# robinhenry/gym-anm

Hardware: AMD Instinct MI355X
Metric: env-steps/sec (whole node) at num_envs=65536, ANM6Easy; NR iters to 1e-6 (higher is better)
Workload: dtype f64

## Files before the change

### gym_anm_amd/csrc/anm_device.hpp

```cpp
#pragma once

#include <cmath>
#include <cstdint>
#include <type_traits>

#if defined(__HIPCC__)
#define ANM_HD __host__ __device__ __forceinline__
#define ANM_CONST_AS __attribute__((address_space(4)))
#else
#define ANM_HD inline
#define ANM_CONST_AS
#endif

#if defined(ANM_PHASE_TIMING) && defined(__HIPCC__)
#define ANM_N_PHASES 8
#define ANM_MAX_WAVES 16384
__device__ unsigned long long g_anm_phase[ANM_N_PHASES][ANM_MAX_WAVES];
#endif
#if defined(ANM_PHASE_TIMING) && defined(__HIP_DEVICE_COMPILE__)
#define ANM_PHASE(k)                                                                         \
  do {                                                                                       \
    if ((threadIdx.x & 63) == 0 && blockIdx.x < ANM_MAX_WAVES)                               \
      g_anm_phase[k][blockIdx.x] = __builtin_readcyclecounter();                             \
  } while (0)
#else
#define ANM_PHASE(k) do { } while (0)
#endif

#if defined(__HIPCC__)
#define ANM_WAVE_SYNC()                                        \
  do {                                                         \
    __builtin_amdgcn_fence(__ATOMIC_RELEASE, "wavefront");     \
    __builtin_amdgcn_wave_barrier();                           \
    __builtin_amdgcn_fence(__ATOMIC_ACQUIRE, "wavefront");     \
  } while (0)
#endif

namespace anm {

typedef const ANM_CONST_AS double* cptr_t;

template <int B, int E, class F>
ANM_HD void static_for(F&& f) {
  if constexpr (B < E) {
    f(std::integral_constant<int, B>{});
    static_for<B + 1, E>(f);
  }
}

#if defined(__HIP_DEVICE_COMPILE__)
#define ANM_WAVE_ANY(x) __any(x)
#else
#define ANM_WAVE_ANY(x) (x)
#endif

enum DevType : int { DEV_LOAD = -1, DEV_SLACK = 0, DEV_CLASSICAL = 1, DEV_RENEWABLE = 2, DEV_STORAGE = 3 };

constexpr double SINCOS_MEDIUM_MAX = 3.5e15;
ANM_HD int lo_word(double x) {
#if defined(__HIP_DEVICE_COMPILE__)
  return __double2loint(x);
#else
  unsigned long long u;
  __builtin_memcpy(&u, &x, 8);
  return int(unsigned(u));
#endif
}
ANM_HD double flip_sign(double x, unsigned m) {
#if defined(__HIP_DEVICE_COMPILE__)
  return __hiloint2double(__double2hiint(x) ^ int(m & 0x80000000u), __double2loint(x));
#else
  unsigned long long u;
  __builtin_memcpy(&u, &x, 8);
  u ^= (unsigned long long)(m & 0x80000000u) << 32;
  __builtin_memcpy(&x, &u, 8);
  return x;
#endif
}

template <bool NEG>
ANM_HD double fma3(double a, double b, double c) {
#if defined(__HIP_DEVICE_COMPILE__)
  double r;
  if constexpr (NEG) asm("v_fma_f64 %0, %1, %2, -%3" : "=v"(r) : "v"(a), "v"(b), "v"(c));
  else asm("v_fma_f64 %0, %1, %2, %3" : "=v"(r) : "v"(a), "v"(b), "v"(c));
  return r;
#else
  return fma(a, b, NEG ? -c : c);
#endif
}

template <bool VCOEF = false>
ANM_HD void sincos_kernel(double r, int q, double& s_out, double& c_out) {
  const double z = r * r;
  double sn, cs;
#if defined(__HIP_DEVICE_COMPILE__)
  if constexpr (VCOEF) {
    double ps, pc;
    asm("v_fma_f64 %0, %2, %3, %4\n\t"
        "v_fma_f64 %1, %2, %9, %10\n\t"
        "v_fma_f64 %0, %2, %0, %5\n\t"
        "v_fma_f64 %1, %2, %1, %11\n\t"
        "v_fma_f64 %0, %2, %0, %6\n\t"
        "v_fma_f64 %1, %2, %1, %12\n\t"
        "v_fma_f64 %0, %2, %0, %7\n\t"
        "v_fma_f64 %1, %2, %1, %13\n\t"
        "v_fma_f64 %0, %2, %0, %8\n\t"
        "v_fma_f64 %1, %2, %1, %14"
        : "=&v"(ps), "=&v"(pc)
        : "v"(z), "v"(1.58969099521155010221e-10), "v"(-2.50507602534068634195e-08), "v"(2.75573137070700676789e-06),
          "v"(-1.98412698298579493134e-04), "v"(8.33333333332248946124e-03), "v"(-1.66666666666666324348e-01),
          "v"(-1.13596475577881948265e-11), "v"(2.08757232129817482790e-09), "v"(-2.75573143513906633035e-07),
          "v"(2.48015872894767294178e-05), "v"(-1.38888888888741095749e-03), "v"(4.16666666666666019037e-02));
    sn = fma(r * z, ps, r);
    cs = fma(z * z, pc, fma(-0.5, z, 1.0));
  } else
#endif
  {
    double ps = fma(z, 1.58969099521155010221e-10, -2.50507602534068634195e-08);
    ps = fma(z, ps, 2.75573137070700676789e-06);
    ps = fma(z, ps, -1.98412698298579493134e-04);
    ps = fma(z, ps, 8.33333333332248946124e-03);
    ps = fma(z, ps, -1.66666666666666324348e-01);
    sn = fma(r * z, ps, r);
    double pc = fma(z, -1.13596475577881948265e-11, 2.08757232129817482790e-09);
    pc = fma(z, pc, -2.75573143513906633035e-07);
    pc = fma(z, pc, 2.48015872894767294178e-05);
    pc = fma(z, pc, -1.38888888888741095749e-03);
    pc = fma(z, pc, 4.16666666666666019037e-02);
    cs = fma(z * z, pc, fma(-0.5, z, 1.0));
  }
  const bool swap = (q & 1) != 0;
  const double a = swap ? cs : sn, b = swap ? sn : cs;
  s_out = flip_sign(a, unsigned(q) << 30);
  c_out = flip_sign(b, unsigned(q + 1) << 30);
}


ANM_HD void reduce_medium(double x, double& r_out, int& q_out) {
  const double TWO_OVER_PI = 6.36619772367581382433e-01;
  const double P1 = 1.57079632679489655800e+00, P2 = 6.12323399573676603587e-17, P3 = 1.49738490485916983e-33;
  const double fn = rint(x * TWO_OVER_PI);
  double r = fma(-fn, P1, x);
  r = fma(-fn, P2, r);
  r = fma(-fn, P3, r);
  const double f2 = rint(r * TWO_OVER_PI);
  r = fma(-f2, P1, r);
  r = fma(-f2, P2, r);
  r_out = r;
  q_out = lo_word((fn + f2) + 6755399441055744.0);
}
struct SinCos {
  double s, c;
};
#if defined(__HIPCC__)
__host__ __device__ __attribute__((noinline))
#else
inline
#endif
SinCos sincos_huge(double x) {
  SinCos r;
  sincos(x, &r.s, &r.c);
  return r;
}

template <bool VCOEF = false>
ANM_HD void sincos_medium(double x, double& s_out, double& c_out) {
  double r;
  int q;
  reduce_medium(x, r, q);
  sincos_kernel<VCOEF>(r, q, s_out, c_out);
}

enum SetDevField : int {
  SD_PMIN = 0, SD_PMAX, SD_QMIN, SD_QMAX,
  SD_SOC_MIN, SD_SOC_MAX, SD_EFF, SD_PAD,
  SD_HLO_LO, SD_HLO_HI,
  SD_HHI_LO, SD_HHI_HI,
  SD_SL,
  SD_SIZE = SD_SL + 4 * 6
};
enum SlField : int { SL_TAU = 0, SL_RHO, SL_INV, SL_LO, SL_HI, SL_SENSE };

template <class T>
struct Layout {
  static constexpr int SCALARS = 0;
  static constexpr int N_SCALARS = 8;
  static constexpr int Y_RE = SCALARS + N_SCALARS;
  static constexpr int Y_IM = Y_RE + T::NNZ;
  static constexpr int BUS_VMIN = Y_IM + T::NNZ;
  static constexpr int BUS_VMAX = BUS_VMIN + T::NB;
  static constexpr int BR = BUS_VMAX + T::NB;
  static constexpr int BR_STRIDE = 9;
  static constexpr int LOAD = BR + T::NBR * BR_STRIDE;
  static constexpr int SETDEV = LOAD + T::NLOAD * 3;
  static constexpr int KMAX = 8;
  static constexpr int OBS_LO = SETDEV + T::NSET * SD_SIZE;
  static constexpr int OBS_HI = OBS_LO + T::SDIM + KMAX;
  static constexpr int TOTAL = OBS_HI + T::SDIM + KMAX;
};
enum ScalarField : int { SC_BASE = 0, SC_DT, SC_LAMB, SC_C1, SC_C2, SC_RTERM, SC_PERIOD, SC_SPARE };

#if defined(__HIP_DEVICE_COMPILE__)
ANM_HD double vmax(double a, double b) { double r; asm("v_max_f64 %0, %1, %2" : "=v"(r) : "v"(a), "v"(b)); return r; }
ANM_HD double vmin(double a, double b) { double r; asm("v_min_f64 %0, %1, %2" : "=v"(r) : "v"(a), "v"(b)); return r; }
#else
ANM_HD double vmax(double a, double b) { return fmax(a, b); }
ANM_HD double vmin(double a, double b) { return fmin(a, b); }
#endif

template <int NSL, class SD>
ANM_HD void project_pq(SD sd, double p0, double q0, double pl, double pu, double& p_out, double& q_out) {
  const double ql = sd[SD_QMIN], qu = sd[SD_QMAX];
  const double EPS = 1e-12;
  double best_d = INFINITY, bp = p0, bq = q0;
  bool any_viol = false;

  auto consider = [&](bool violated, bool valid, double cp, double cq) {
    any_viol = any_viol || violated;
    const double dp = cp - p0, dq = cq - q0;
    const double d = dp * dp + dq * dq;
    const bool take = violated && valid && (d < best_d);
    best_d = take ? d : best_d;
    bp = take ? cp : bp;
    bq = take ? cq : bq;
  };

  auto vertical = [&](bool violated, double c) {
    double lo = ql, hi = qu;
    static_for<0, NSL>([&](auto K) {
      constexpr int k = K;
      const double tau = sd[SD_SL + 6 * k + SL_TAU], rho = sd[SD_SL + 6 * k + SL_RHO];
      const double sense = sd[SD_SL + 6 * k + SL_SENSE];
      const double v = tau * c + rho;
      hi = (sense > 0.0) ? vmin(hi, v) : hi;
      lo = (sense < 0.0) ? vmax(lo, v) : lo;
    });
    const bool valid = lo <= hi + EPS;
    const double t = vmin(vmax(q0, lo), hi);
    consider(violated, valid, c, t);
  };
  vertical(p0 < pl, pl);
  vertical(p0 > pu, pu);

  auto horizontal = [&](bool violated, double c, double slo, double shi) {
    const double lo = vmax(pl, slo), hi = vmin(pu, shi);
    const bool valid = lo <= hi + EPS;
    const double t = vmin(vmax(p0, lo), hi);
    consider(violated, valid, t, c);
  };
  horizontal(q0 < ql, ql, sd[SD_HLO_LO], sd[SD_HLO_HI]);
  horizontal(q0 > qu, qu, sd[SD_HHI_LO], sd[SD_HHI_HI]);

  static_for<0, NSL>([&](auto K) {
    constexpr int k = K;
    const double tau = sd[SD_SL + 6 * k + SL_TAU], rho = sd[SD_SL + 6 * k + SL_RHO];
    const double inv = sd[SD_SL + 6 * k + SL_INV], sense = sd[SD_SL + 6 * k + SL_SENSE];
    const double line = tau * p0 + rho;
    const bool violated = (sense > 0.0) ? (q0 > line) : ((sense < 0.0) ? (q0 < line) : false);
    const double lo = vmax(pl, sd[SD_SL + 6 * k + SL_LO]), hi = vmin(pu, sd[SD_SL + 6 * k + SL_HI]);
    const bool valid = lo <= hi + EPS;
    const double ts = (p0 + tau * (q0 - rho)) * inv;
    const double t = vmin(vmax(ts, lo), hi);
    consider(violated, valid, t, tau * t + rho);
  });

  p_out = any_viol ? bp : p0;
  q_out = any_viol ? bq : q0;
}

template <class R>
struct Blk {
  R a, b, c, d;
};

ANM_HD double recip(double x) {
#if defined(__HIP_DEVICE_COMPILE__)
  double r = __builtin_amdgcn_rcp(x);
  r = r * fma(-x, r, 2.0);
  r = r * fma(-x, r, 2.0);
  return __hiloint2double(fabs(x) < 2.2250738585072014e-308 ? 0x7ff80000 : __double2hiint(r), __double2loint(r));
#else
  return 1.0 / x;
#endif
}
ANM_HD float recip(float x) { return 1.0f / x; }

ANM_HD double dump_div(double num, double den) {
#if defined(__HIP_DEVICE_COMPILE__)
  double r = __builtin_amdgcn_rcp(den);
  r = r * fma(-den, r, 2.0);
  r = r * fma(-den, r, 2.0);
  const double q = num * r;
  return fma(fma(-den, q, num), r, q);
#else
  return num / den;
#endif
}
struct Recip {
  double d, r;
};
ANM_HD Recip make_recip(double d) {
#if defined(__HIP_DEVICE_COMPILE__)
  return Recip{d, recip(d)};
#else
  return Recip{d, 1.0 / d};
#endif
}
ANM_HD double div_by(double x, const Recip& k) {
#if defined(__HIP_DEVICE_COMPILE__)
  const double q = x * k.r;
  return __builtin_amdgcn_div_fixup(fma(fma(-k.d, q, x), k.r, q), k.d, x);
#else
  return x / k.d;
#endif
}
ANM_HD double dump_abs(double x, double y) { return sqrt(fma(x, x, y * y)); }
ANM_HD double dump_arg(double y, double x) {
  const double ax = fabs(x), ay = fabs(y);
  const bool swap = ay > ax;
  const double m1 = swap ? ay : ax, m0 = swap ? ax : ay;
  const int up = m1 < 0x1p-900 ? 200 : 0;
  const double mx = ldexp(m1, up), mn = ldexp(m0, up);
  const bool big = mn > 0.41421356237309503 * mx;
  const double t = dump_div(big ? mn - mx : mn, big ? mn + mx : mx);
  const double s = t * t;
  double p = -2.54135080938672937e-02;
  p = fma(p, s, 5.03577166688385092e-02);
  p = fma(p, s, -6.51081127522272901e-02);
  p = fma(p, s, 7.67463247369439688e-02);
  p = fma(p, s, -9.08967227312245662e-02);
  p = fma(p, s, 1.11110596251928595e-01);
  p = fma(p, s, -1.42857131220131439e-01);
  p = fma(p, s, 1.99999999884144603e-01);
  p = fma(p, s, -3.33333333333071968e-01);
  p = fma(p, s, 1.00000000000000022e+00);
  double a = t * p;
  a = big ? a + 0.78539816339744828 : a;
  a = swap ? 1.5707963267948966 - a : a;
  a = (x < 0.0) ? 3.1415926535897931 - a : a;
  a = (mx == 0.0) ? (std::signbit(x) ? 3.1415926535897931 : 0.0) : a;
  return copysign(a, y);
}
ANM_HD double dump_signed_abs(double re, double mag) { return fma(0.0, mag, re); }

ANM_HD double fm(double a, double b, double c) { return fma(a, b, c); }
ANM_HD float fm(float a, float b, float c) { return fmaf(a, b, c); }

template <class R>
ANM_HD Blk<R> blk_inv(const Blk<R>& m) {
  const R det = fm(m.a, m.d, -(m.b * m.c));
  const R r = recip(det);
  return Blk<R>{m.d * r, -m.b * r, -m.c * r, m.a * r};
}
template <class R>
ANM_HD Blk<R> blk_mul(const Blk<R>& x, const Blk<R>& y) {
  return Blk<R>{fm(x.a, y.a, x.b * y.c), fm(x.a, y.b, x.b * y.d), fm(x.c, y.a, x.d * y.c), fm(x.c, y.b, x.d * y.d)};
}
template <class R>
ANM_HD void blk_submul(Blk<R>& z, const Blk<R>& x, const Blk<R>& y) {
  z.a = fm(-x.b, y.c, fm(-x.a, y.a, z.a));
  z.b = fm(-x.b, y.d, fm(-x.a, y.b, z.b));
  z.c = fm(-x.d, y.c, fm(-x.c, y.a, z.c));
  z.d = fm(-x.d, y.d, fm(-x.c, y.b, z.d));
}

template <class T>
struct EnvWork {
  double dev_p[T::ND], dev_q[T::ND];
  double p_pot[T::NGEN > 0 ? T::NGEN : 1];
  double soc[T::NDES > 0 ? T::NDES : 1];
  double bus_p[T::NB], bus_q[T::NB];
  double vm[T::NB];
  double vr[T::NB], vi[T::NB];
  double ir[T::NB], ii[T::NB];
  int n_iter;
  double diff;
  bool converged;
  double e_loss, penalty, reward;
  double br_pf[T::NBR], br_qf[T::NBR], br_pt[T::NBR], br_qt[T::NBR], br_s[T::NBR];
  double br_ifr[T::NBR], br_ifi[T::NBR];
};

template <class T>
ANM_HD void update_angles(const double (&dth)[T::NB], double (&cs)[T::NB], double (&sn)[T::NB]) {
  double dmax = 0.0;
  static_for<1, T::NB>([&](auto I) { dmax = fmax(dmax, fabs(dth[I])); });
  const bool small_step = dmax <= 0.78;
  if (!ANM_WAVE_ANY(!small_step)) {
    static_for<1, T::NB>([&](auto I) {
      constexpr int i = I;
      double sd, cd;
      sincos_kernel(dth[i], 0, sd, cd);
      const double c = cs[i], s = sn[i];
      cs[i] = fma(c, cd, s * sd);
      sn[i] = fma(s, cd, -(c * sd));
    });
    return;
  }
  if (dmax < SINCOS_MEDIUM_MAX) {
    static_for<1, T::NB>([&](auto I) {
      constexpr int i = I;
      double r, sd, cd;
      int q;
      reduce_medium(dth[i], r, q);
      sincos_kernel(r, q, sd, cd);
      const double c = cs[i], s = sn[i];
      cs[i] = fma(c, cd, s * sd);
      sn[i] = fma(s, cd, -(c * sd));
    });
  } else {
    static_for<1, T::NB>([&](auto I) {
      constexpr int i = I;
      const SinCos r = sincos_huge(dth[i]);
      const double c = cs[i], s = sn[i];
      cs[i] = fma(c, r.c, s * r.s);
      sn[i] = fma(s, r.c, -(c * r.s));
    });
  }
}

template <class T>
struct PFState {
  double cs[T::NB], sn[T::NB];
  int it;
  double diff;
  bool active;
  bool fresh;
};

template <class T>
constexpr int y_transposed(int z) {
  for (int t = 0; t < T::NNZ; ++t)
    if (T::Y_I[t] == T::Y_J[z] && T::Y_J[t] == T::Y_I[z]) return t;
  return -1;
}

template <class T>
ANM_HD double eval_mismatch(cptr_t C, EnvWork<T>& w, const double (&cs)[T::NB], const double (&sn)[T::NB],
                            double (&wr)[T::NNZ], double (&wi)[T::NNZ], double (&sr)[T::NB], double (&si)[T::NB]) {
  typedef Layout<T> L;
  w.vr[0] = 1.0;
  w.vi[0] = 0.0;
  static_for<1, T::NB>([&](auto I) {
    constexpr int i = I;
    w.vr[i] = w.vm[i] * cs[i];
    w.vi[i] = w.vm[i] * sn[i];
  });
  static_for<0, T::NNZ>([&](auto Z) {
    constexpr int z = Z;
    constexpr int i = T::Y_I[z], k = T::Y_J[z];
    if constexpr (i >= 1) {
      const double yr = C[L::Y_RE + z], yi = C[L::Y_IM + z];
      if constexpr (k == 0) {
        wr[z] = fma(w.vr[i], yr, w.vi[i] * yi);
        wi[z] = fma(w.vi[i], yr, -(w.vr[i] * yi));
      } else if constexpr (k == i) {
        const double m2 = w.vm[i] * w.vm[i];
        wr[z] = yr * m2;
        wi[z] = -(yi * m2);
      } else if constexpr (i < k) {
        constexpr int zt = y_transposed<T>(z);
        static_assert(zt >= 0, "the sparsity pattern of Y must be structurally symmetric");
        const double pr = fma(w.vr[i], w.vr[k], w.vi[i] * w.vi[k]);
        const double pi = fma(w.vi[i], w.vr[k], -(w.vr[i] * w.vi[k]));
        wr[z] = fma(yr, pr, yi * pi);
        wi[z] = fma(yr, pi, -(yi * pr));
        const double tr = C[L::Y_RE + zt], ti = C[L::Y_IM + zt];
        wr[zt] = fma(tr, pr, -(ti * pi));
        wi[zt] = -fma(tr, pi, ti * pr);
      }
    }
  });
  static_for<0, T::NNZ>([&](auto Z) {
    constexpr int z = Z;
    constexpr int i = T::Y_I[z];
    if constexpr (i >= 1) {
      constexpr bool first = (z == 0) || (T::Y_I[z > 0 ? z - 1 : 0] != i);
      if constexpr (first) {
        sr[i] = wr[z];
        si[i] = wi[z];
      } else {
        sr[i] += wr[z];
        si[i] += wi[z];
      }
    }
  });
  double nrm = 0.0;
  bool isnan_ = false;
  static_for<1, T::NB>([&](auto I) {
    constexpr int i = I;
    const double a = fabs(sr[i] - w.bus_p[i]), b = fabs(si[i] - w.bus_q[i]);
    isnan_ = isnan_ || (a != a) || (b != b);
    nrm = fmax(nrm, fmax(a, b));
  });
  return isnan_ ? NAN : nrm;
}

template <class T, class JT>
ANM_HD void newton_update(EnvWork<T>& w, double (&cs)[T::NB], double (&sn)[T::NB], const double (&wr_)[T::NNZ],
                          const double (&wi_)[T::NNZ], const double (&sr)[T::NB], const double (&si)[T::NB],
                          bool active) {
  Blk<JT> J[T::NBLK];
  JT r0[T::NB], r1[T::NB];
  static_for<1, T::NB>([&](auto I) {
    constexpr int i = I;
    r0[i] = JT(sr[i] - w.bus_p[i]);
    r1[i] = JT(si[i] - w.bus_q[i]);
  });
  static_for<0, T::NFILL>([&](auto Fz) {
    constexpr int b = T::FILL_BLK[Fz];
    J[b] = Blk<JT>{JT(0), JT(0), JT(0), JT(0)};
  });
  static_for<0, T::NNZ>([&](auto Z) {
    constexpr int z = Z;
    constexpr int i = T::Y_I[z], k = T::Y_J[z];
    constexpr int b = T::YBLK[z];
    if constexpr (b >= 0) {
      const double wr = wr_[z], wi = wi_[z];
      if constexpr (i == k) {
        J[b] = Blk<JT>{JT(-(si[i] - wi)), JT(sr[i] + wr), JT(sr[i] - wr), JT(si[i] + wi)};
      } else {
        J[b] = Blk<JT>{JT(wi), JT(wr), JT(-wr), JT(wi)};
      }
    }
  });

  static_for<0, T::NU>([&](auto KS) {
    constexpr int ks = KS;
    constexpr int k = T::PIV[ks];
    constexpr int dk = T::DIAG[k];
    J[dk] = blk_inv(J[dk]);
    static_for<T::LSEG[ks], T::LSEG[ks + 1]>([&](auto LI) {
      constexpr int l = LI;
      constexpr int i = T::L_I[l];
      constexpr int bl = T::L_BLK[l];
      const Blk<JT> Lik = blk_mul(J[bl], J[dk]);
      J[bl] = Lik;
      r0[i] = fm(-Lik.b, r1[k], fm(-Lik.a, r0[k], r0[i]));
      r1[i] = fm(-Lik.d, r1[k], fm(-Lik.c, r0[k], r1[i]));
      static_for<T::USEG[l], T::USEG[l + 1]>([&](auto UI) {
        constexpr int u = UI;
        blk_submul(J[T::U_DST[u]], Lik, J[T::U_SRC[u]]);
      });
    });
  });
  JT d0[T::NB], d1[T::NB];
  static_for<0, T::NU>([&](auto KR) {
    constexpr int ks = T::NU - 1 - KR;
    constexpr int k = T::PIV[ks];
    JT a0 = r0[k], a1 = r1[k];
    static_for<T::BSEG[ks], T::BSEG[ks + 1]>([&](auto BI) {
      constexpr int s = BI;
      constexpr int j = T::B_J[s];
      const Blk<JT>& U = J[T::B_BLK[s]];
      a0 = fm(-U.b, d1[j], fm(-U.a, d0[j], a0));
      a1 = fm(-U.d, d1[j], fm(-U.c, d0[j], a1));
    });
    const Blk<JT>& Di = J[T::DIAG[k]];
    d0[k] = fm(Di.a, a0, Di.b * a1);
    d1[k] = fm(Di.c, a0, Di.d * a1);
  });
  if (active) {
    double dth[T::NB];
    static_for<1, T::NB>([&](auto I) {
      constexpr int i = I;
      dth[i] = double(d0[i]);
      w.vm[i] = fma(-double(d1[i]), fabs(w.vm[i]), w.vm[i]);
    });
    update_angles<T>(dth, cs, sn);
  }
}

template <class T>
ANM_HD void pf_begin(EnvWork<T>& w, PFState<T>& st) {
  static_for<0, T::NB>([&](auto I) {
    constexpr int i = I;
    w.vm[i] = 1.0;
    st.cs[i] = 1.0;
    st.sn[i] = 0.0;
  });
  st.it = 0;
  st.diff = 0.0;
  st.active = false;
  st.fresh = true;
}

template <class T>
ANM_HD void pf_idle(PFState<T>& st) {
  st.it = 0;
  st.diff = 0.0;
  st.active = false;
  st.fresh = false;
}

template <class T, class JT>
ANM_HD void pf_iterate(cptr_t C, EnvWork<T>& w, PFState<T>& st, double tol, int max_iter, int iter_cap) {
  bool inc = false;
  bool take = st.fresh;
  ANM_PHASE(2);
  while (true) {
    double wr[T::NNZ], wi[T::NNZ], sr[T::NB], si[T::NB];
    const double nd = eval_mismatch<T>(C, w, st.cs, st.sn, wr, wi, sr, si);
    st.it = inc ? st.it + 1 : st.it;
    st.diff = take ? nd : st.diff;
    st.active = (st.diff > tol) && (st.it < max_iter);
    const bool run = st.active && (st.it < iter_cap);
    if (!ANM_WAVE_ANY(run)) break;
    newton_update<T, JT>(w, st.cs, st.sn, wr, wi, sr, si, run);
    inc = take = run;
  }
  st.fresh = false;
  ANM_PHASE(3);
}

template <class T>
ANM_HD void pf_end(cptr_t C, EnvWork<T>& w, const PFState<T>& st, double tol) {
  typedef Layout<T> L;
  ANM_PHASE(4);
  w.n_iter = st.it;
  w.diff = st.diff;
  const bool conv = !(st.diff != st.diff);
  w.converged = conv && (st.diff <= tol);
  static_for<0, T::NNZ>([&](auto Z) {
    constexpr int z = Z;
    constexpr int i = T::Y_I[z], j = T::Y_J[z];
    const double yr = C[L::Y_RE + z], yi = C[L::Y_IM + z];
    const double tr = fma(yr, w.vr[j], -(yi * w.vi[j])), ti = fma(yr, w.vi[j], yi * w.vr[j]);
    constexpr bool first = (z == 0) || (T::Y_I[z > 0 ? z - 1 : 0] != i);
    if constexpr (first) {
      w.ir[i] = tr;
      w.ii[i] = ti;
    } else {
      w.ir[i] += tr;
      w.ii[i] += ti;
    }
  });
  const double s0r = w.ir[0], s0i = -w.ii[0];
  w.bus_p[0] = (s0r != s0r) ? INFINITY : s0r;
  w.bus_q[0] = (s0i != s0i) ? INFINITY : s0i;
}

template <class T>
ANM_HD void flows_and_reward(cptr_t C, EnvWork<T>& w) {
  typedef Layout<T> L;
  const double dt = C[L::SCALARS + SC_DT], lamb = C[L::SCALARS + SC_LAMB];
  double pen = 0.0;
  static_for<0, T::NBR>([&](auto Bi) {
    constexpr int b = Bi;
    constexpr int f = T::BR_F[b], t = T::BR_T[b];
    cptr_t c = C + L::BR + b * L::BR_STRIDE;
    const double ifr = c[0] * w.vr[f] - c[1] * w.vi[f] + c[2] * w.vr[t] - c[3] * w.vi[t];
    const double ifi = c[0] * w.vi[f] + c[1] * w.vr[f] + c[2] * w.vi[t] + c[3] * w.vr[t];
    const double itr = c[4] * w.vr[t] - c[5] * w.vi[t] + c[6] * w.vr[f] - c[7] * w.vi[f];
    const double iti = c[4] * w.vi[t] + c[5] * w.vr[t] + c[6] * w.vi[f] + c[7] * w.vr[f];
    const double pf = w.vr[f] * ifr + w.vi[f] * ifi, qf = w.vi[f] * ifr - w.vr[f] * ifi;
    const double pt = w.vr[t] * itr + w.vi[t] * iti, qt = w.vi[t] * itr - w.vr[t] * iti;
    const double sf2 = pf * pf + qf * qf, st2 = pt * pt + qt * qt;
    const double sg = (pf > 0.0) ? 1.0 : ((pf < 0.0) ? -1.0 : ((pf == 0.0) ? 0.0 : NAN));
    const double smax = (sf2 != sf2 || st2 != st2) ? NAN : sqrt(vmax(sf2, st2));
    const double s = sg * smax;
    w.br_pf[b] = pf; w.br_qf[b] = qf; w.br_pt[b] = pt; w.br_qt[b] = qt; w.br_s[b] = s;
    w.br_ifr[b] = ifr; w.br_ifi[b] = ifi;
    const double over = fabs(s) - c[8];
    pen += (over != over) ? NAN : fmax(0.0, over);
  });
  static_for<0, T::NB>([&](auto I) {
    constexpr int i = I;
    const double vmag = (i == 0) ? 1.0 : fabs(w.vm[i]);
    const double hi = vmag - C[L::BUS_VMAX + i], lo = C[L::BUS_VMIN + i] - vmag;
    pen += (vmag != vmag) ? NAN : (fmax(0.0, hi) + fmax(0.0, lo));
  });
  double e = 0.0;
  static_for<0, T::ND>([&](auto Di) {
    constexpr int d = Di;
    constexpr int typ = T::DEV_TYPE[d];
    if constexpr (typ != DEV_STORAGE) e += w.dev_p[d];
    if constexpr (typ == DEV_RENEWABLE) {
      const double curt = w.p_pot[T::DEV_SLOT[d]] - w.dev_p[d];
      e += (curt != curt) ? NAN : fmax(0.0, curt);
    }
  });
  w.e_loss = e * dt;
  w.penalty = pen * (dt * lamb);
  w.reward = -(w.e_loss + w.penalty);
}

template <class T, class JT, class CD>
ANM_HD void transition_begin(cptr_t C, CD Cd, EnvWork<T>& w, PFState<T>& st,
                             const double (&P_load)[T::NLOAD > 0 ? T::NLOAD : 1],
                             const double (&P_pot)[T::NGEN > 0 ? T::NGEN : 1],
                             const double (&P_set)[T::NSET > 0 ? T::NSET : 1],
                             const double (&Q_set)[T::NSET > 0 ? T::NSET : 1], double tol, int max_iter, int iter_cap) {
  typedef Layout<T> L;
  const double dt = C[L::SCALARS + SC_DT];
  const Recip base = make_recip(C[L::SCALARS + SC_BASE]);
  static_for<0, T::ND>([&](auto Di) {
    constexpr int d = Di;
    constexpr int typ = T::DEV_TYPE[d];
    if constexpr (typ == DEV_LOAD) {
      constexpr int s = T::DEV_SLOT[d];
      auto c = Cd + L::LOAD + 3 * s;
      const double p = vmin(vmax(div_by(P_load[s], base), c[0]), c[1]);
      w.dev_p[d] = p;
      w.dev_q[d] = p * c[2];
    } else if constexpr (typ == DEV_CLASSICAL || typ == DEV_RENEWABLE) {
      constexpr int g = T::DEV_SLOT[d], s = T::DEV_SET[d];
      auto sd = Cd + L::SETDEV + SD_SIZE * s;
      const double pp = vmin(vmax(div_by(P_pot[g], base), sd[SD_PMIN]), sd[SD_PMAX]);
      w.p_pot[g] = pp;
      project_pq<2>(sd, div_by(P_set[s], base), div_by(Q_set[s], base), sd[SD_PMIN], vmin(pp, sd[SD_PMAX]), w.dev_p[d],
                                      w.dev_q[d]);
    } else if constexpr (typ == DEV_STORAGE) {
      constexpr int e = T::DEV_SLOT[d], s = T::DEV_SET[d];
      auto sd = Cd + L::SETDEV + SD_SIZE * s;
      const double soc = w.soc[e], eff = sd[SD_EFF];
      const double s_lo = (soc - sd[SD_SOC_MAX]) / (dt * eff);
      const double s_hi = eff * (soc - sd[SD_SOC_MIN]) / dt;
      project_pq<4>(sd, div_by(P_set[s], base), div_by(Q_set[s], base), vmax(s_lo, sd[SD_PMIN]), vmin(s_hi, sd[SD_PMAX]),
                                      w.dev_p[d], w.dev_q[d]);
      const double p = w.dev_p[d];
      const double ns = (p <= 0.0) ? (soc - dt * eff * p) : (soc - dt * p / eff);
      w.soc[e] = vmin(vmax(ns, sd[SD_SOC_MIN]), sd[SD_SOC_MAX]);
    } else {
      w.dev_p[d] = 0.0;
      w.dev_q[d] = 0.0;
    }
  });
  static_for<0, T::NB>([&](auto I) {
    constexpr int i = I;
    w.bus_p[i] = 0.0;
    w.bus_q[i] = 0.0;
  });
  static_for<0, T::ND>([&](auto Di) {
    constexpr int d = Di;
    constexpr int b = T::DEV_BUS[d];
    w.bus_p[b] += w.dev_p[d];
    w.bus_q[b] += w.dev_q[d];
  });
  pf_begin<T>(w, st);
  if (iter_cap >= 0) pf_iterate<T, JT>(C, w, st, tol, max_iter, iter_cap);
}

template <class T>
ANM_HD void transition_end(cptr_t C, EnvWork<T>& w, const PFState<T>& st, double tol) {
  pf_end<T>(C, w, st, tol);
  static_for<0, T::ND>([&](auto Di) {
    constexpr int d = Di;
    if constexpr (T::DEV_TYPE[d] == DEV_SLACK) {
      w.dev_p[d] = w.bus_p[T::DEV_BUS[d]];
      w.dev_q[d] = w.bus_q[T::DEV_BUS[d]];
    }
  });
  flows_and_reward<T>(C, w);
  ANM_PHASE(5);
}

template <class T, class JT>
ANM_HD void transition(cptr_t C, EnvWork<T>& w, const double (&P_load)[T::NLOAD > 0 ? T::NLOAD : 1],
                       const double (&P_pot)[T::NGEN > 0 ? T::NGEN : 1],
                       const double (&P_set)[T::NSET > 0 ? T::NSET : 1],
                       const double (&Q_set)[T::NSET > 0 ? T::NSET : 1], double tol, int max_iter) {
  PFState<T> st;
  transition_begin<T, JT>(C, C, w, st, P_load, P_pot, P_set, Q_set, tol, max_iter, max_iter);
  transition_end<T>(C, w, st, tol);
}

struct Philox {
  uint32_t c[4];
  ANM_HD static void round(uint32_t (&c)[4], uint32_t k0, uint32_t k1) {
    const uint64_t p0 = uint64_t(0xD2511F53u) * c[0];
    const uint64_t p1 = uint64_t(0xCD9E8D57u) * c[2];
    const uint32_t n0 = uint32_t(p1 >> 32) ^ c[1] ^ k0;
    const uint32_t n1 = uint32_t(p1);
    const uint32_t n2 = uint32_t(p0 >> 32) ^ c[3] ^ k1;
    const uint32_t n3 = uint32_t(p0);
    c[0] = n0; c[1] = n1; c[2] = n2; c[3] = n3;
  }
  ANM_HD static void generate(uint64_t seed, uint64_t env, uint32_t epoch, uint32_t draw, uint32_t (&out)[4]) {
    uint32_t c[4] = {uint32_t(env), uint32_t(env >> 32), epoch, draw};
    uint32_t k0 = uint32_t(seed), k1 = uint32_t(seed >> 32);
    for (int r = 0; r < 10; ++r) {
      round(c, k0, k1);
      k0 += 0x9E3779B9u;
      k1 += 0xBB67AE85u;
    }
    out[0] = c[0]; out[1] = c[1]; out[2] = c[2]; out[3] = c[3];
  }
  ANM_HD static double u01(uint32_t hi, uint32_t lo) {
    const uint64_t v = ((uint64_t(hi) << 32) | lo) >> 11;
    return double(v) * (1.0 / 9007199254740992.0);
  }
  ANM_HD static double u01_of(const uint32_t (&q)[4], int u) {
    const bool odd = (u & 1) != 0;
    return u01(odd ? q[2] : q[0], odd ? q[3] : q[1]);
  }
  ANM_HD static double unit_u01(uint64_t seed, uint64_t env, uint32_t epoch, int u) {
    uint32_t q[4];
    generate(seed, env, epoch, 1u + u / 2, q);
    return u01_of(q, u);
  }
};

struct ExoUniform {
  static constexpr uint32_t KEY_DRAW = 0xFFFFFFFFu, TAG = 0x45584F31u;
  ANM_HD static uint64_t episode_key(uint64_t seed, uint64_t env, uint32_t epoch) {
    uint32_t r[4];
    Philox::generate(seed, env, epoch, KEY_DRAW, r);
    return uint64_t(r[0]) | (uint64_t(r[1]) << 32);
  }
  ANM_HD static void block(uint64_t key, uint32_t t, uint32_t j, uint32_t (&q)[4]) {
    Philox::generate(key, uint64_t(t) | (uint64_t(j) << 32), 0u, TAG, q);
  }
  ANM_HD static double map(double lo, double hi, double u) { return fma(hi - lo, u, lo); }
  ANM_HD static double draw(uint64_t key, uint32_t t, int i, double lo, double hi) {
    uint32_t q[4];
    block(key, t, uint32_t(i) >> 1, q);
    return map(lo, hi, Philox::u01_of(q, i));
  }
};

struct ExoNoise {
  ANM_HD static double map(double amp, double w, double mean, double lo, double hi) {
    const double x = fma(amp, w, mean);
    return x < lo ? lo : (x > hi ? hi : x);
  }
  ANM_HD static double factor(const uint32_t (&q)[4], int i) { return fma(2.0, Philox::u01_of(q, i), -1.0); }
  ANM_HD static double draw(uint64_t key, uint32_t t, int i, double amp, double mean, double lo, double hi) {
    uint32_t q[4];
    ExoUniform::block(key, t, uint32_t(i) >> 1, q);
    return map(amp, factor(q, i), mean, lo, hi);
  }
  ANM_HD static double advance(double rho, double c, double z, double w) {
    const double t = c * w;
    return fma(rho, z, t);
  }
  ANM_HD static double map_state(double amp, double z, double mean, double lo, double hi) { return map(amp, z, mean, lo, hi); }
  template <class Put>
  ANM_HD static void forecast_row(double rho, double z, const double* amp, const double* mean, double lo, double hi, int aux,
                                  int period, int H, Put&& put) {
    int at = (aux + 1) % period;
    if (at < 0) at += period;
    for (int i = 0; i < H; ++i) {
      z = advance(rho, 1.0, z, 0.0);
      put(i, map_state(amp[at], z, mean[at], lo, hi));
      if (++at == period) at = 0;
    }
  }
};

template <class T>
struct FullState {
  static constexpr int BUS_P = 0, BUS_Q = BUS_P + T::NB, BUS_VM = BUS_Q + T::NB, BUS_VA = BUS_VM + T::NB,
                       BUS_IM = BUS_VA + T::NB, BUS_IA = BUS_IM + T::NB, DEV_P = BUS_IA + T::NB,
                       DEV_Q = DEV_P + T::ND, DES_SOC = DEV_Q + T::ND, GEN_PMAX = DES_SOC + T::NDES,
                       BR_P = GEN_PMAX + T::NGEN, BR_Q = BR_P + T::NBR, BR_S = BR_Q + T::NBR,
                       BR_IM = BR_S + T::NBR, BR_IA = BR_IM + T::NBR, SIZE = BR_IA + T::NBR;
};

enum FullClass : unsigned { FC_BUS_P = 0, FC_BUS_Q, FC_BUS_VM, FC_BUS_VA, FC_BUS_IM, FC_BUS_IA, FC_DEV_P, FC_DEV_Q, FC_DES_SOC,
                            FC_GEN_PMAX, FC_BR_P, FC_BR_Q, FC_BR_S, FC_BR_IM, FC_BR_IA, FC_COUNT };

template <class T, class Put>
ANM_HD void emit_full_state(const EnvWork<T>& w, unsigned need, Put&& put) {
  auto want = [&](unsigned c) { return (need >> c) & 1u; };
  if (want(FC_BUS_P)) static_for<0, T::NB>([&](auto I) { put(FC_BUS_P, I, w.bus_p[I]); });
  if (want(FC_BUS_Q)) static_for<0, T::NB>([&](auto I) { put(FC_BUS_Q, I, w.bus_q[I]); });
  if (want(FC_BUS_VM)) static_for<0, T::NB>([&](auto I) { put(FC_BUS_VM, I, dump_abs(w.vr[I], w.vi[I])); });
  if (want(FC_BUS_VA)) static_for<0, T::NB>([&](auto I) { put(FC_BUS_VA, I, dump_arg(w.vi[I], w.vr[I])); });
  if (want(FC_BUS_IM)) static_for<0, T::NB>([&](auto I) { put(FC_BUS_IM, I, dump_abs(w.ir[I], w.ii[I])); });
  if (want(FC_BUS_IA)) static_for<0, T::NB>([&](auto I) { put(FC_BUS_IA, I, dump_arg(w.ii[I], w.ir[I])); });
  if (want(FC_DEV_P)) static_for<0, T::ND>([&](auto D) { put(FC_DEV_P, D, w.dev_p[D]); });
  if (want(FC_DEV_Q)) static_for<0, T::ND>([&](auto D) { put(FC_DEV_Q, D, w.dev_q[D]); });
  if (want(FC_DES_SOC)) static_for<0, T::NDES>([&](auto E) { put(FC_DES_SOC, E, w.soc[E]); });
  if (want(FC_GEN_PMAX)) static_for<0, T::NGEN>([&](auto G) { put(FC_GEN_PMAX, G, w.p_pot[G]); });
  if (want(FC_BR_P)) static_for<0, T::NBR>([&](auto B) { put(FC_BR_P, B, w.br_pf[B]); });
  if (want(FC_BR_Q)) static_for<0, T::NBR>([&](auto B) { put(FC_BR_Q, B, w.br_qf[B]); });
  if (want(FC_BR_S)) static_for<0, T::NBR>([&](auto B) { put(FC_BR_S, B, w.br_s[B]); });
  if (want(FC_BR_IM))
    static_for<0, T::NBR>([&](auto Bi) {
      constexpr int b = Bi;
      put(FC_BR_IM, b, dump_signed_abs(w.br_ifr[b], dump_abs(w.br_ifr[b], w.br_ifi[b])));
    });
  if (want(FC_BR_IA)) static_for<0, T::NBR>([&](auto B) { put(FC_BR_IA, B, dump_arg(w.br_ifi[B], w.br_ifr[B])); });
}

template <class T>
ANM_HD constexpr int full_class_base(unsigned c) {
  typedef FullState<T> F;
  constexpr int base[FC_COUNT] = {F::BUS_P, F::BUS_Q, F::BUS_VM, F::BUS_VA, F::BUS_IM, F::BUS_IA, F::DEV_P, F::DEV_Q,
                                  F::DES_SOC, F::GEN_PMAX, F::BR_P, F::BR_Q, F::BR_S, F::BR_IM, F::BR_IA};
  return base[c];
}

struct FullOffsets {
  int base[FC_COUNT + 1];
};
constexpr FullOffsets full_offsets(int NB, int ND, int NDES, int NGEN, int NBR) {
  const int width[FC_COUNT] = {NB, NB, NB, NB, NB, NB, ND, ND, NDES, NGEN, NBR, NBR, NBR, NBR, NBR};
  FullOffsets o{};
  for (unsigned c = 0; c < FC_COUNT; ++c) o.base[c + 1] = o.base[c] + width[c];
  return o;
}
template <class T>
constexpr bool full_offsets_match() {
  const FullOffsets o = full_offsets(T::NB, T::ND, T::NDES, T::NGEN, T::NBR);
  for (unsigned c = 0; c < FC_COUNT; ++c)
    if (o.base[c] != full_class_base<T>(c)) return false;
  return o.base[FC_COUNT] == FullState<T>::SIZE;
}
template <class D>
void set_full_offsets(D& d) {
  const FullOffsets o = full_offsets(d.NB, d.ND, d.NDES, d.NGEN, d.NBR);
  d.f_bus_p = o.base[FC_BUS_P]; d.f_bus_q = o.base[FC_BUS_Q]; d.f_bus_vm = o.base[FC_BUS_VM]; d.f_bus_va = o.base[FC_BUS_VA];
  d.f_bus_im = o.base[FC_BUS_IM]; d.f_bus_ia = o.base[FC_BUS_IA]; d.f_dev_p = o.base[FC_DEV_P]; d.f_dev_q = o.base[FC_DEV_Q];
  d.f_des_soc = o.base[FC_DES_SOC]; d.f_gen_pmax = o.base[FC_GEN_PMAX]; d.f_br_p = o.base[FC_BR_P]; d.f_br_q = o.base[FC_BR_Q];
  d.f_br_s = o.base[FC_BR_S]; d.f_br_im = o.base[FC_BR_IM]; d.f_br_ia = o.base[FC_BR_IA]; d.FS = o.base[FC_COUNT];
}

template <class T>
ANM_HD void write_full_state(const EnvWork<T>& w, double* out) {
  emit_full_state<T>(w, ~0u, [&](unsigned c, int i, double v) { out[full_class_base<T>(c) + i] = v; });
}

}
```

Before: 1.062 billion.

## Micro-optimize Newton power-flow loop with register-resident sincos coefficients and lane early-exit

Reworks the inner Newton iteration in several ways. Sincos polynomial coefficients are kept in VGPRs for mid-sized networks, and quadrant selection becomes branchless bit masking. Huge-angle handling turns into a wave-uniform fixup over the medium path, and the mismatch norm uses fused abs-max asm. Inactive lanes now skip the Jacobian solve, and voltage writes to the work struct move out of the loop into a single post-loop store. The aim is fewer instructions, scalar constant loads and memory stores per iteration, at the cost of higher register pressure and an extra explicit waitcnt.

```diff
diff --git a/gym_anm_amd/csrc/anm_device.hpp b/gym_anm_amd/csrc/anm_device.hpp
--- a/gym_anm_amd/csrc/anm_device.hpp
+++ b/gym_anm_amd/csrc/anm_device.hpp
@@ -57,6 +57,7 @@
 enum DevType : int { DEV_LOAD = -1, DEV_SLACK = 0, DEV_CLASSICAL = 1, DEV_RENEWABLE = 2, DEV_STORAGE = 3 };
 
 constexpr double SINCOS_MEDIUM_MAX = 3.5e15;
+constexpr int SINCOS_VCOEF_MIN_NB = 5, SINCOS_VCOEF_MAX_NB = 8;
 ANM_HD int lo_word(double x) {
 #if defined(__HIP_DEVICE_COMPILE__)
   return __double2loint(x);
@@ -78,6 +79,23 @@
 #endif
 }
 
+ANM_HD int spread_bit0(int q) {
+#if defined(__HIP_DEVICE_COMPILE__)
+  int m;
+  asm("v_bfe_i32 %0, %1, 0, 1" : "=v"(m) : "v"(q));
+  return m;
+#else
+  return -(q & 1);
+#endif
+}
+ANM_HD double pick_bits(double x, double y, int m) {
+#if defined(__HIP_DEVICE_COMPILE__)
+  return __hiloint2double((__double2hiint(x) & ~m) | (__double2hiint(y) & m), (__double2loint(x) & ~m) | (__double2loint(y) & m));
+#else
+  return m ? y : x;
+#endif
+}
+
 template <bool NEG>
 ANM_HD double fma3(double a, double b, double c) {
 #if defined(__HIP_DEVICE_COMPILE__)
@@ -87,6 +105,41 @@
   return r;
 #else
   return fma(a, b, NEG ? -c : c);
+#endif
+}
+template <bool NEG>
+ANM_HD void fma3_into(double& x, double b, double c) {
+#if defined(__HIP_DEVICE_COMPILE__)
+  if constexpr (NEG) asm("v_fma_f64 %0, %0, %1, -%2" : "+v"(x) : "v"(b), "v"(c));
+  else asm("v_fma_f64 %0, %0, %1, %2" : "+v"(x) : "v"(b), "v"(c));
+#else
+  x = fma(x, b, NEG ? -c : c);
+#endif
+}
+ANM_HD double max_abs(double x, double y) {
+#if defined(__HIP_DEVICE_COMPILE__)
+  double t;
+  asm("v_max_f64 %0, |%1|, |%2|" : "=v"(t) : "v"(x), "v"(y));
+  return t;
+#else
+  return fmax(fabs(x), fabs(y));
+#endif
+}
+ANM_HD double max_abs_into(double n, double x, double y) {
+#if defined(__HIP_DEVICE_COMPILE__)
+  double t;
+  asm("v_max_f64 %0, |%1|, |%2|\n\tv_max_f64 %0, %3, %0" : "=&v"(t) : "v"(x), "v"(y), "v"(n));
+  return t;
+#else
+  return fmax(n, fmax(fabs(x), fabs(y)));
+#endif
+}
+ANM_HD double step_magnitude(double d, double v) {
+#if defined(__HIP_DEVICE_COMPILE__)
+  asm("v_fma_f64 %0, -%1, |%0|, %0" : "+v"(v) : "v"(d));
+  return v;
+#else
+  return fma(-d, fabs(v), v);
 #endif
 }
 
@@ -136,6 +189,88 @@
   c_out = flip_sign(b, unsigned(q + 1) << 30);
 }
 
+struct SinCosCoef {
+  double s[6], c[6];
+};
+ANM_HD SinCosCoef sincos_coef() {
+  return SinCosCoef{{1.58969099521155010221e-10, -2.50507602534068634195e-08, 2.75573137070700676789e-06,
+                     -1.98412698298579493134e-04, 8.33333333332248946124e-03, -1.66666666666666324348e-01},
+                    {-1.13596475577881948265e-11, 2.08757232129817482790e-09, -2.75573143513906633035e-07,
+                     2.48015872894767294178e-05, -1.38888888888741095749e-03, 4.16666666666666019037e-02}};
+}
+ANM_HD SinCosCoef sincos_coef_resident() {
+  SinCosCoef k = sincos_coef();
+#if defined(__HIP_DEVICE_COMPILE__)
+#pragma unroll
+  for (int i = 0; i < 6; ++i) {
+    asm("" : "+v"(k.s[i]));
+    asm("" : "+v"(k.c[i]));
+  }
+#endif
+  return k;
+}
+
+ANM_HD void sincos_small(double r, double& sn, double& cs, const SinCosCoef& k) {
+  const double z = r * r;
+#if defined(__HIP_DEVICE_COMPILE__)
+  double t, u;
+  asm("v_fma_f64 %0, %4, %5, %6\n\t"
+      "v_fma_f64 %1, %4, %11, %12\n\t"
+      "v_fma_f64 %0, %4, %0, %7\n\t"
+      "v_fma_f64 %1, %4, %1, %13\n\t"
+      "v_fma_f64 %0, %4, %0, %8\n\t"
+      "v_fma_f64 %1, %4, %1, %14\n\t"
+      "v_fma_f64 %0, %4, %0, %9\n\t"
+      "v_fma_f64 %1, %4, %1, %15\n\t"
+      "v_fma_f64 %0, %4, %0, %10\n\t"
+      "v_fma_f64 %1, %4, %1, %16\n\t"
+      "v_mul_f64 %2, %17, %4\n\t"
+      "v_fma_f64 %3, %4, -0.5, 1.0\n\t"
+      "v_fma_f64 %0, %2, %0, %17\n\t"
+      "v_mul_f64 %2, %4, %4\n\t"
+      "v_fma_f64 %1, %2, %1, %3"
+      : "=&v"(sn), "=&v"(cs), "=&v"(t), "=&v"(u)
+      : "v"(z), "v"(k.s[0]), "v"(k.s[1]), "v"(k.s[2]), "v"(k.s[3]), "v"(k.s[4]), "v"(k.s[5]),
+        "v"(k.c[0]), "v"(k.c[1]), "v"(k.c[2]), "v"(k.c[3]), "v"(k.c[4]), "v"(k.c[5]), "v"(r));
+#else
+  double ps = fma(z, k.s[0], k.s[1]);
+  static_for<2, 6>([&](auto I) { ps = fma(z, ps, k.s[I]); });
+  double pc = fma(z, k.c[0], k.c[1]);
+  static_for<2, 6>([&](auto I) { pc = fma(z, pc, k.c[I]); });
+  sn = fma(r * z, ps, r);
+  cs = fma(z * z, pc, fma(-0.5, z, 1.0));
+#endif
+}
+struct SinCosLiteral {};
+ANM_HD void sincos_small(double r, double& sn, double& cs, SinCosLiteral) {
+  const double z = r * r;
+  double ps = fma(z, 1.58969099521155010221e-10, -2.50507602534068634195e-08);
+  ps = fma(z, ps, 2.75573137070700676789e-06);
+  ps = fma(z, ps, -1.98412698298579493134e-04);
+  ps = fma(z, ps, 8.33333333332248946124e-03);
+  ps = fma(z, ps, -1.66666666666666324348e-01);
+  sn = fma(r * z, ps, r);
+  double pc = fma(z, -1.13596475577881948265e-11, 2.08757232129817482790e-09);
+  pc = fma(z, pc, -2.75573143513906633035e-07);
+  pc = fma(z, pc, 2.48015872894767294178e-05);
+  pc = fma(z, pc, -1.38888888888741095749e-03);
+  pc = fma(z, pc, 4.16666666666666019037e-02);
+  cs = fma(z * z, pc, fma(-0.5, z, 1.0));
+}
+
+ANM_HD void sincos_quadrant(double sn, double cs, int q, double& s_out, double& c_out) {
+  const int odd = spread_bit0(q);
+  const double a = pick_bits(sn, cs, odd), b = pick_bits(cs, sn, odd);
+  s_out = flip_sign(a, unsigned(q) << 30);
+  c_out = flip_sign(b, unsigned(q + 1) << 30);
+}
+template <class K>
+ANM_HD void sincos_kernel(double r, int q, double& s_out, double& c_out, const K& k) {
+  double sn, cs;
+  sincos_small(r, sn, cs, k);
+  sincos_quadrant(sn, cs, q, s_out, c_out);
+}
+
 
 ANM_HD void reduce_medium(double x, double& r_out, int& q_out) {
   const double TWO_OVER_PI = 6.36619772367581382433e-01;
@@ -170,6 +305,13 @@
   int q;
   reduce_medium(x, r, q);
   sincos_kernel<VCOEF>(r, q, s_out, c_out);
+}
+template <class K>
+ANM_HD void sincos_medium(double x, double& s_out, double& c_out, const K& k) {
+  double r;
+  int q;
+  reduce_medium(x, r, q);
+  sincos_kernel(r, q, s_out, c_out, k);
 }
 
 enum SetDevField : int {
@@ -382,42 +524,31 @@
   double br_ifr[T::NBR], br_ifi[T::NBR];
 };
 
-template <class T>
-ANM_HD void update_angles(const double (&dth)[T::NB], double (&cs)[T::NB], double (&sn)[T::NB]) {
+template <class T, class K>
+ANM_HD void update_angles(const double (&dth)[T::NB], double (&cs)[T::NB], double (&sn)[T::NB], const K& k) {
   double dmax = 0.0;
   static_for<1, T::NB>([&](auto I) { dmax = fmax(dmax, fabs(dth[I])); });
   const bool small_step = dmax <= 0.78;
+  double sd[T::NB], cd[T::NB];
   if (!ANM_WAVE_ANY(!small_step)) {
-    static_for<1, T::NB>([&](auto I) {
-      constexpr int i = I;
-      double sd, cd;
-      sincos_kernel(dth[i], 0, sd, cd);
-      const double c = cs[i], s = sn[i];
-      cs[i] = fma(c, cd, s * sd);
-      sn[i] = fma(s, cd, -(c * sd));
-    });
-    return;
-  }
-  if (dmax < SINCOS_MEDIUM_MAX) {
-    static_for<1, T::NB>([&](auto I) {
-      constexpr int i = I;
-      double r, sd, cd;
-      int q;
-      reduce_medium(dth[i], r, q);
-      sincos_kernel(r, q, sd, cd);
-      const double c = cs[i], s = sn[i];
-      cs[i] = fma(c, cd, s * sd);
-      sn[i] = fma(s, cd, -(c * sd));
-    });
+    static_for<1, T::NB>([&](auto I) { sincos_small(dth[I], sd[I], cd[I], k); });
   } else {
-    static_for<1, T::NB>([&](auto I) {
-      constexpr int i = I;
-      const SinCos r = sincos_huge(dth[i]);
-      const double c = cs[i], s = sn[i];
-      cs[i] = fma(c, r.c, s * r.s);
-      sn[i] = fma(s, r.c, -(c * r.s));
-    });
-  }
+    const bool huge = !(dmax < SINCOS_MEDIUM_MAX);
+    static_for<1, T::NB>([&](auto I) { sincos_medium(dth[I], sd[I], cd[I], k); });
+    if (ANM_WAVE_ANY(huge)) {
+      static_for<1, T::NB>([&](auto I) {
+        const SinCos r = sincos_huge(dth[I]);
+        sd[I] = huge ? r.s : sd[I];
+        cd[I] = huge ? r.c : cd[I];
+      });
+    }
+  }
+  static_for<1, T::NB>([&](auto I) {
+    constexpr int i = I;
+    const double t1 = sn[i] * sd[i], t2 = cs[i] * sd[i];
+    fma3_into<false>(cs[i], cd[i], t1);
+    fma3_into<true>(sn[i], cd[i], t2);
+  });
 }
 
 template <class T>
@@ -437,16 +568,28 @@
 }
 
 template <class T>
-ANM_HD double eval_mismatch(cptr_t C, EnvWork<T>& w, const double (&cs)[T::NB], const double (&sn)[T::NB],
+ANM_HD void iterate_voltage(const EnvWork<T>& w, const double (&cs)[T::NB], const double (&sn)[T::NB], double (&vr)[T::NB],
+                            double (&vi)[T::NB]) {
+  vr[0] = 1.0;
+  vi[0] = 0.0;
+  static_for<1, T::NB>([&](auto I) {
+    constexpr int i = I;
+    vr[i] = w.vm[i] * cs[i];
+    vi[i] = w.vm[i] * sn[i];
+  });
+}
+
+template <class T>
+ANM_HD double eval_mismatch(cptr_t C, const EnvWork<T>& w_, const double (&cs)[T::NB], const double (&sn)[T::NB],
                             double (&wr)[T::NNZ], double (&wi)[T::NNZ], double (&sr)[T::NB], double (&si)[T::NB]) {
   typedef Layout<T> L;
-  w.vr[0] = 1.0;
-  w.vi[0] = 0.0;
-  static_for<1, T::NB>([&](auto I) {
-    constexpr int i = I;
-    w.vr[i] = w.vm[i] * cs[i];
-    w.vi[i] = w.vm[i] * sn[i];
-  });
+  struct {
+    double vr[T::NB], vi[T::NB];
+    const double (&vm)[T::NB];
+    const double (&bus_p)[T::NB];
+    const double (&bus_q)[T::NB];
+  } w{{}, {}, w_.vm, w_.bus_p, w_.bus_q};
+  iterate_voltage<T>(w_, cs, sn, w.vr, w.vi);
   static_for<0, T::NNZ>([&](auto Z) {
     constexpr int z = Z;
     constexpr int i = T::Y_I[z], k = T::Y_J[z];
@@ -490,17 +633,19 @@
   bool isnan_ = false;
   static_for<1, T::NB>([&](auto I) {
     constexpr int i = I;
-    const double a = fabs(sr[i] - w.bus_p[i]), b = fabs(si[i] - w.bus_q[i]);
-    isnan_ = isnan_ || (a != a) || (b != b);
-    nrm = fmax(nrm, fmax(a, b));
+    const double fr = sr[i] - w.bus_p[i], fi = si[i] - w.bus_q[i];
+    isnan_ = isnan_ || __builtin_isunordered(fr, fi);
+    if constexpr (i == 1) nrm = max_abs(fr, fi);
+    else nrm = max_abs_into(nrm, fr, fi);
   });
   return isnan_ ? NAN : nrm;
 }
 
-template <class T, class JT>
+template <class T, class JT, class K>
 ANM_HD void newton_update(EnvWork<T>& w, double (&cs)[T::NB], double (&sn)[T::NB], const double (&wr_)[T::NNZ],
                           const double (&wi_)[T::NNZ], const double (&sr)[T::NB], const double (&si)[T::NB],
-                          bool active) {
+                          bool active, const K& k) {
+  if (!active) return;
   Blk<JT> J[T::NBLK];
   JT r0[T::NB], r1[T::NB];
   static_for<1, T::NB>([&](auto I) {
@@ -561,15 +706,13 @@
     d0[k] = fm(Di.a, a0, Di.b * a1);
     d1[k] = fm(Di.c, a0, Di.d * a1);
   });
-  if (active) {
-    double dth[T::NB];
-    static_for<1, T::NB>([&](auto I) {
-      constexpr int i = I;
-      dth[i] = double(d0[i]);
-      w.vm[i] = fma(-double(d1[i]), fabs(w.vm[i]), w.vm[i]);
-    });
-    update_angles<T>(dth, cs, sn);
-  }
+  double dth[T::NB];
+  static_for<1, T::NB>([&](auto I) {
+    constexpr int i = I;
+    dth[i] = double(d0[i]);
+    w.vm[i] = step_magnitude(double(d1[i]), w.vm[i]);
+  });
+  update_angles<T>(dth, cs, sn, k);
 }
 
 template <class T>
@@ -599,17 +742,25 @@
   bool inc = false;
   bool take = st.fresh;
   ANM_PHASE(2);
-  while (true) {
+#if defined(__HIP_DEVICE_COMPILE__)
+  __builtin_amdgcn_s_waitcnt(0xC07F);
+#endif
+  typedef std::conditional_t<(T::NB >= SINCOS_VCOEF_MIN_NB && T::NB <= SINCOS_VCOEF_MAX_NB), SinCosCoef, SinCosLiteral> K;
+  K k{};
+  if constexpr (std::is_same<K, SinCosCoef>::value) k = sincos_coef_resident();
+  bool go;
+  do {
     double wr[T::NNZ], wi[T::NNZ], sr[T::NB], si[T::NB];
     const double nd = eval_mismatch<T>(C, w, st.cs, st.sn, wr, wi, sr, si);
     st.it = inc ? st.it + 1 : st.it;
     st.diff = take ? nd : st.diff;
     st.active = (st.diff > tol) && (st.it < max_iter);
     const bool run = st.active && (st.it < iter_cap);
-    if (!ANM_WAVE_ANY(run)) break;
-    newton_update<T, JT>(w, st.cs, st.sn, wr, wi, sr, si, run);
+    go = ANM_WAVE_ANY(run);
+    newton_update<T, JT>(w, st.cs, st.sn, wr, wi, sr, si, run, k);
     inc = take = run;
-  }
+  } while (go);
+  iterate_voltage<T>(w, st.cs, st.sn, w.vr, w.vi);
   st.fresh = false;
   ANM_PHASE(3);
 }
```

Measured after the change: 1.065 billion (median of 6 runs). Within noise of the previous version (+0.3%).
